# voyage-ai/weaviate

Hardware: AMD Instinct MI355X
Metric: exact kNN QPS (k=10) at 1/2/4/8 GPUs; % of HBM-BW or MFMA roofline (higher is better)
Workload: dtype f32 (exact result; int8 MFMA block-key filter); 1 GPU; 10M x 768 fp32 cosine, k=10, exact flat search (BASELINE configs[2]); corpus_rows=10000000, dims=768, k=10, query_batch=8192, parallelism=corpus sharded over 1 GPU(s), contiguous id ranges, replayed_queries=240

## Files before the change

### weaviate_amd/csrc/q8_kernels.hip

```cpp
#pragma once
#include "batch_row.h"

namespace wv {
namespace {

typedef int i32x4_t __attribute__((ext_vector_type(4)));
typedef int i32x16_t __attribute__((ext_vector_type(16)));
constexpr int Q8_NONE = (int)0x80000000;


template <int OFF>
__device__ __forceinline__ i32x4_t lds_ld16_o(unsigned base) {
    i32x4_t v;
    asm volatile("ds_read_b128 %0, %1 offset:%2" : "=v"(v) : "v"(base), "i"(OFF));
    return v;
}

__global__ void k_allow_bits(const uint64_t* __restrict__ ids, int64_t n, uint64_t id_base, int64_t hiwater,
                             const uint32_t* __restrict__ present, uint32_t* __restrict__ bits,
                             uint32_t* __restrict__ cnt) {
    const int64_t i = (int64_t)blockIdx.x * blockDim.x + threadIdx.x;
    if (i >= n) return;
    const uint64_t id = ids[i];
    if (id < id_base || id - id_base >= (uint64_t)hiwater) return;
// ... 205 lines not shown
        sh += __shfl_xor(sh, o);
        sr += __shfl_xor(sr, o);
    }
    if (lane == 0) {
        const float4 q16 = qinfo16[q];
        qscale[q] = sq;
        qinfo8[q] = make_float4(q16.x, sh, sr, (bad || q16.w != 0.f || !(sh < 1e30f)) ? 1.f : 0.f);
    }
}

}
struct Q8Args {
    const unsigned char* X8;
    const float* sb;
    const float* xnorm2;
    const uint32_t* valid;
    const unsigned char* Q8;
    const float* qscale;
    float* key;
    int64_t ldk;
    int64_t nslots;
    int slots_per_span;
    int nspans;
    int nqg;
    int bq_bits;
    int64_t nq_live = 1ll << 62;
    int prio = 0;
    const uint32_t* qmask = nullptr;
    int64_t qmask_ld = 0;
    int64_t qmask_n = 1;
};
namespace {

template <int NC, int RB, bool ISL2, bool STAG = false, bool BQ = false, int PF = 1, int DBG = 0, bool LIVE = false,
          bool MASK = false>
__global__ __launch_bounds__(512, 2) void k_q8_blockkey(Q8Args a) {
    constexpr int NPB = 2 * NC;
    constexpr int SLOT = RB * NPB * 1024;
    constexpr int P = RB * NPB / 8;
    static_assert((RB * NPB) % 8 == 0, "pieces per slot must split over 8 waves");
    static_assert(RB == 1 || RB == 2, "RB must be 1 or 2");
    constexpr int64_t TILE_B = (int64_t)NPB * 8192;
    constexpr int NT = RB * NC;
    constexpr int P0 = P + 2 + (ISL2 ? 1 : 0) + (MASK ? 1 : 0);
    static_assert(P0 < NC, "the deferred key store must follow the slot's DMA pieces");
    static_assert(PF >= 1 && PF + 1 < NC, "prefetch distance");
    static_assert(!STAG || RB == 2, "the stagger defers a slot's second block");
    static_assert(!BQ || (!ISL2 && !STAG), "BQ: integer maxima, in-order schedule");
    static_assert(!LIVE || (RB == 2 && !STAG && !BQ && DBG == 0), "LIVE: the paired in-order schedule");
    static_assert(!MASK || (RB == 2 && !STAG && !BQ && !ISL2 && DBG == 0), "MASK: paired dot / cosine keys");
    constexpr int X0 = 1;
    constexpr int XE = 2 + (ISL2 ? 2 * RB : 0) + (MASK ? 2 : 0);
    constexpr int NBUF = 3;
    extern __shared__ __attribute__((aligned(16))) unsigned char qsm[];

    const int tid = threadIdx.x;
    const int lane = tid & 63;
    const int wave = __builtin_amdgcn_readfirstlane(tid >> 6);
    const int total = a.nqg * a.nspans;
    const int b = blockIdx.x;
    const int logical = (total % 8 == 0) ? (b % 8) * (total / 8) + (b / 8) : b;
    const int span = logical / a.nqg, grp = logical % a.nqg;
    const bool act = !LIVE || (int64_t)grp * 256 + wave * 32 < a.nq_live;

    i32x4_t Qf[2 * NC];
    const int64_t q0 = (int64_t)grp * 256 + wave * 32;
    if (act) {
        const int j = lane & 15, kq = lane >> 4;
        const unsigned char* qp =
            a.Q8 + (int64_t)grp * TILE_B + (kq >> 1) * 8192 + (wave * 32 + j) * 32 + 16 * (kq & 1);
#pragma unroll
        for (int c = 0; c < NC; c++)
#pragma unroll
            for (int n = 0; n < 2; n++)
                Qf[2 * c + n] = *reinterpret_cast<const i32x4_t*>(qp + (2 * c) * 8192 + n * 16 * 32);
    }
    const float sqA = BQ ? 1.f : a.qscale[q0 + (lane & 15)];
    const float sqB = BQ ? 1.f : a.qscale[q0 + 16 + (lane & 15)];
    constexpr bool PAIR = RB == 2 && !STAG;
    const float sqO = (BQ || !PAIR) ? 1.f : a.qscale[q0 + (lane & 15) + 16 * (lane >> 5)];
    __builtin_amdgcn_s_waitcnt(0x0F70);

    const int64_t s0 = (int64_t)span * a.slots_per_span;
// ... 201 lines not shown
        } else if constexpr (ISL2) {
            float p0, p1;
            reduce(ac, vw_, sb_, xa_, xb_, p0, p1);
            rr[0] = __float_as_uint(p0);
            rr[1] = __float_as_uint(p1);
        } else if (vw == 0xFFFFFFFFu) {
#pragma unroll
            for (int n = 0; n < 2; n++)
                rr[n] = (uint32_t)max(max(max(ac[0][n][0], ac[0][n][1]), max(ac[0][n][2], ac[0][n][3])),
                                      max(max(ac[1][n][0], ac[1][n][1]), max(ac[1][n][2], ac[1][n][3])));
        } else {
#pragma unroll
            for (int n = 0; n < 2; n++) {
                int mi = Q8_NONE;
#pragma unroll
                for (int mm = 0; mm < 2; mm++)
#pragma unroll
                    for (int r = 0; r < 4; r++) mi = max(mi, ((vl >> (16 * mm + r)) & 1u) ? ac[mm][n][r] : Q8_NONE);
                rr[n] = (uint32_t)mi;
            }
        }
        r0 = rr[0];
        r1 = rr[1];
    };
    constexpr uint32_t PNONE = ISL2 ? 0x7f800000u : (uint32_t)Q8_NONE;
    uint32_t pA0 = PNONE, pA1 = PNONE, pB0 = PNONE, pB1 = PNONE;
    float psA = 0.f, psB = 0.f;
    i32x4_t acc[RB][2][2];
    const bool late = STAG && wave >= 4;
    uint32_t dvw = 0;
    float dsb = 0.f;
    f32x4_t dxa = {0.f, 0.f, 0.f, 0.f}, dxb = {0.f, 0.f, 0.f, 0.f};
    if (a.prio && wave >= 4) __builtin_amdgcn_s_setprio(1);
    auto slot_loop = [&](auto actc) {
    constexpr bool ACT = decltype(actc)::value;
    int cur = 0;
    for (int t = 0; t < nsteps; t++) {
        const int nxt = cur == NBUF - 1 ? 0 : cur + 1;
        const int gslot = cur == 0 ? NBUF - 1 : cur - 1;
        const unsigned sbase = ring + (unsigned)(cur * SLOT) + l16;
        const int dma = __builtin_amdgcn_readfirstlane(t + 2 < nsteps ? 1 : 0);
        const unsigned sm = (unsigned)(t & 3);
        uint2 vwv;
        float2 sbv;
        uint2 mw0 = uint2{0u, 0u}, mw1 = uint2{0u, 0u};
        f32x4_t xa[RB], xb[RB];
        if constexpr (!ISL2) {
#pragma unroll
            for (int r = 0; r < RB; r++) xa[r] = xb[r] = f32x4_t{0.f, 0.f, 0.f, 0.f};
        }
        static_for<0, NT>([&](auto ttc) {
            constexpr int tt = decltype(ttc)::value;
            constexpr int rb = tt / NC, c = tt % NC;
            if constexpr (tt == X0 && ACT) {
                asm volatile("ds_read_b64 %0, %1" : "=v"(vwv) : "v"(vring + sm * 16u));
                asm volatile("ds_read_b64 %0, %1" : "=v"(sbv) : "v"(sring + sm * 16u));
                if constexpr (MASK) {
                    const unsigned mb = mring + sm * 256u + (unsigned)((lane & 15) * 8);
                    asm volatile("ds_read_b64 %0, %1" : "=v"(mw0) : "v"(mb));
                    asm volatile("ds_read_b64 %0, %1 offset:128" : "=v"(mw1) : "v"(mb));
                }
                if constexpr (ISL2) {
                    const unsigned xbase = xnring + sm * (unsigned)(RB * 128) + (unsigned)(16 * ((lane >> 4) & 3));
                    xa[0] = lds_ld4f_o<0>(xbase);
                    xb[0] = lds_ld4f_o<64>(xbase);
                    if constexpr (RB == 2) {
// ... 67 lines not shown
            dsb = sbv.y;
            dxa = xa[RB - 1];
            dxb = xb[RB - 1];
        } else if constexpr (PAIR && !(DBG & 4)) {
            if constexpr (ACT) {
                reduce_raw(acc[1], vwv.y, sbv.y, xa[1], xb[1], pB0, pB1, mw1);
                psA = sbv.x;
                psB = sbv.y;
            }
        } else if constexpr (!(DBG & 4)) {
            reduce(acc[RB - 1], RB == 2 ? vwv.y : vwv.x, RB == 2 ? sbv.y : sbv.x, xa[RB - 1], xb[RB - 1], mp0, mp1);
        } else {
#pragma unroll
            for (int r = 0; r < RB; r++)
                dbg_sink ^= acc[r][0][0][0] ^ acc[r][0][1][0] ^ acc[r][1][0][0] ^ acc[r][1][1][0];
        }
        gbp = (s0 + t) * RB + (PAIR ? 0 : RB - 1);
        if (t + 1 < nsteps) {
            if constexpr (DBG != 0) {
                qs_wait_vm_c<0>();
            } else if (t >= 2 && t + 2 < nsteps) {
                qs_wait_vm_c<2 * SPS + P0>();
            } else {
                const int y = (t >= 1 ? stores_in(t - 1) : 0) + stores_in(t) + (t + 2 < nsteps ? P0 : 0);
                qs_wait_vm(y);
            }
            __builtin_amdgcn_s_barrier();
            __builtin_amdgcn_sched_barrier(0);
            if constexpr (ACT) head_reads(ring + (unsigned)(nxt * SLOT) + l16);
        }
        cur = nxt;
    }
    };
    if constexpr (LIVE) {
        if (act) slot_loop(std::true_type{});
        else slot_loop(std::false_type{});
    } else {
        slot_loop(std::true_type{});
    }
    if (nsteps > 0 && !(DBG & 4)) {
        if constexpr (PAIR) {
            finish2(pA0, pA1, pB0, pB1, psA, psB, gbp);
        } else {
            if (late) reduce(acc[RB - 1], dvw, dsb, dxa, dxb, mp0, mp1);
            finish(mp0, mp1, gbp);
        }
    }
    if constexpr ((DBG & 12) != 0) {
        if (a.ldk == -1234567) krow[0] = (float)dbg_sink;
    }
}

template <int NC, int RB, bool ISL2>
__global__ __launch_bounds__(512, 2) void k_q8_blockkey32(Q8Args a) {
    constexpr int SLOT = RB * NC * 1024;
    constexpr int P = RB * NC / 8;
    static_assert((RB * NC) % 8 == 0, "pieces per slot must split over 8 waves");
    constexpr int64_t TILE_B = (int64_t)NC * 8192;
    constexpr int NBUF = 3;
    extern __shared__ __attribute__((aligned(16))) unsigned char qsm[];

    const int tid = threadIdx.x;
    const int lane = tid & 63;
    const int wave = __builtin_amdgcn_readfirstlane(tid >> 6);
    const int li = lane & 31, lh = lane >> 5;
    const int total = a.nqg * a.nspans;
    const int b = blockIdx.x;
    const int logical = (total % 8 == 0) ? (b % 8) * (total / 8) + (b / 8) : b;
    const int span = logical / a.nqg, grp = logical % a.nqg;

    i32x4_t Qf[NC];
    {
        const unsigned char* qp = a.Q8 + (int64_t)grp * TILE_B + (wave * 32 + li) * 32 + 16 * lh;
#pragma unroll
// ... 450 lines not shown
```

### weaviate_amd/csrc/qs_runtime.hip

```cpp
#include "rt_index.h"

int qs_R(int k) { return k + 1 <= 64 ? 2 : k + 1 <= 192 ? 4 : k + 1 <= 448 ? 8 : k + 1 <= 960 ? 16 : 0; }
int qs_R_flat(int k) {
    const int r = qs_R(k);
    return r ? r : k + 1 <= 1984 ? 32 : k + 1 <= 4032 ? 64 : 0;
}

int invert_lists(wv_index* idx, hipStream_t s, const uint32_t* cand, const int32_t* ncand, const int32_t* flags,
                 int64_t cn, int L, int64_t nb) {
    HIPCHK(idx->bmCnt.ensure((size_t)nb * sizeof(uint32_t)));
    HIPCHK(idx->bmOff.ensure((size_t)(nb + 1) * sizeof(uint32_t)));
    HIPCHK(idx->bmPairs.ensure((size_t)cn * L * sizeof(uint32_t)));
    if (idx->bmCnt_zp != idx->bmCnt.p || idx->bmCnt_zb != idx->bmCnt.bytes)
        HIPCHK(hipMemsetAsync(idx->bmCnt.p, 0, idx->bmCnt.bytes, s));
    idx->bmCnt_zp = nullptr;
    const unsigned gw = (unsigned)((cn + 3) / 4);
    k_inv_count<<<gw, 256, 0, s>>>(cand, ncand, flags, (int)cn, L, idx->bmCnt.as<uint32_t>());
    const unsigned nparts = (unsigned)((nb + INV_CHUNK - 1) / INV_CHUNK);
    HIPCHK(idx->bmPart.ensure((size_t)nparts * sizeof(uint32_t)));
    k_inv_part<<<nparts, 1024, 0, s>>>(idx->bmCnt.as<uint32_t>(), nb, idx->bmPart.as<uint32_t>());
    k_inv_scan<<<nparts, 1024, 0, s>>>(idx->bmCnt.as<uint32_t>(), nb, idx->bmPart.as<uint32_t>(),
                                       idx->bmOff.as<uint32_t>());
    k_inv_scatter<<<gw, 256, 0, s>>>(cand, ncand, flags, (int)cn, L, idx->bmOff.as<uint32_t>(),
                                     idx->bmCnt.as<uint32_t>(), idx->bmPairs.as<uint32_t>());
    HIPCHK(hipGetLastError());
    idx->bmCnt_zp = idx->bmCnt.p;
    idx->bmCnt_zb = idx->bmCnt.bytes;
    return WV_OK;
}

int launch_q8_keys(wv_index* idx, hipStream_t s, Q8Args a, int dpb8, bool l2) {
    const int NC8 = dpb8 / 64;
    const int RB = dpb8 <= 768 ? 2 : 1;
    int64_t nspans = 256 / std::gcd(256, a.nqg);
    while ((int64_t)a.nqg * nspans < 256) nspans *= 2;
    if (idx->spans_opt > 0) nspans = idx->spans_opt;
    const int64_t max_sps = ((1ll << 32) - 2 * 256ll * dpb8) / ((int64_t)RB * 32 * dpb8);
    nspans = std::max<int64_t>(nspans, (a.nslots + max_sps - 1) / max_sps);
    if (idx->spans_opt <= 0) {
        const int64_t unit = 256 / std::gcd(256, a.nqg);
        nspans = (nspans + unit - 1) / unit * unit;
    }
    nspans = std::max<int64_t>(1, std::min<int64_t>(nspans, a.nslots));
    const int64_t sps = (a.nslots + nspans - 1) / nspans;
    a.slots_per_span = (int)sps;
    a.nspans = (int)((a.nslots + sps - 1) / sps);
    const size_t lds = (size_t)3 * RB * 2 * NC8 * 1024 + 1024 + (l2 ? (size_t)8 * 4 * RB * 128 : 0);
    dim3 grid((unsigned)((int64_t)a.nqg * a.nspans));
#define WV_Q8K(NCV, RBV, L2V)                                                                                  \
    do {                                                                                                       \
        HIPCHK(hipFuncSetAttribute((const void*)k_q8_blockkey<NCV, RBV, L2V, false, false, 1>,                 \
                                   hipFuncAttributeMaxDynamicSharedMemorySize, (int)lds));                     \
        k_q8_blockkey<NCV, RBV, L2V, false, false, 1><<<grid, 512, lds, s>>>(a);                                \
    } while (0)
#define WV_Q8KN(L2V)                                   \
    switch (NC8) {                                     \
    case 8: WV_Q8K(8, 2, L2V); break;                  \
    case 10: WV_Q8K(10, 2, L2V); break;                \
    case 12: WV_Q8K(12, 2, L2V); break;                \
    case 16: WV_Q8K(16, 1, L2V); break;                \
    case 20: WV_Q8K(20, 1, L2V); break;                \
    case 24: WV_Q8K(24, 1, L2V); break;                \
    default: return set_err(WV_ERR_UNSUPPORTED, "int8 keys: plane width %d", dpb8); \
    }
    if (l2) { WV_Q8KN(true); } else { WV_Q8KN(false); }
#undef WV_Q8KN
#undef WV_Q8K
    HIPCHK(hipGetLastError());
    return WV_OK;
}

bool pqa_keys_route(const wv_index* idx) {
    const bool q8 = idx->q8_planes && (idx->q8_opt || idx->q8_only);
    return idx->pqa_keys && q8 && !idx->q8_only && idx->dpb8 <= 768 && idx->metric != WV_METRIC_L2_SQUARED &&
           !idx->q8_stag && idx->q8_shape != 32 && idx->sel_dbg <= 0;
}

int search_qs(wv_index* idx, hipStream_t s, int64_t nq, int k, int mode, const uint32_t* valid,
                     uint64_t* o_ids, float* o_d, int32_t* o_n, int32_t* o_flags, int phase,
                     float* topA, const float* gA, const float* gE, int W) {
    const int kout = mode == 1 ? k + 1 : k;
    const int NK = idx->dpb / 16;
    const bool q8 = idx->q8_planes && (idx->q8_opt || idx->q8_only);
    const bool q8cp = q8 && idx->q8_only;
    const bool q8wide = q8cp && idx->dpb8 > Q8_MAX_DPB;
    const int NC8 = idx->dpb8 / 64;
    const int RB8 = idx->dpb8 <= 768 ? 2 : 1;
    const int RB = q8 ? RB8 : qs_rb(NK);
    const bool pqa = idx->pqa_valid != nullptr;
    const bool pqk = pqa && pqa_keys_route(idx);
    const bool pqs = pqa && !pqk;
    int R = qs_R_flat(k);
    if (q8) {
        if (idx->q8_R > 0) R = std::max(R, idx->q8_R);
        else R = std::max(R, 8);
    }
    if (pqs) R = std::max(R, idx->pqa_R);
    const int L = 64 * (R - 1);
    const int64_t nslots = std::max<int64_t>(1, (idx->hiwater + 32 * RB - 1) / (32 * RB));
// ... 105 lines not shown
        if (time_it) HIPCHK(hipEventRecord(idx->ev0, s));
#define WV_QS(NKV, L2V)                                                                                        \
    do {                                                                                                       \
        HIPCHK(hipFuncSetAttribute((const void*)k_qs_blockkey<NKV, L2V>, hipFuncAttributeMaxDynamicSharedMemorySize, (int)lds)); \
        k_qs_blockkey<NKV, L2V><<<grid, 512, lds, s>>>(a);                                                     \
    } while (0)
#define WV_QS3(NKV, L2V, D)                                                                                    \
    do {                                                                                                       \
        HIPCHK(hipFuncSetAttribute((const void*)k_qs_blockkey<NKV, L2V, D>, hipFuncAttributeMaxDynamicSharedMemorySize, (int)lds)); \
        k_qs_blockkey<NKV, L2V, D><<<grid, 512, lds, s>>>(a);                                                  \
    } while (0)
#define WV_QSN(L2V)                                    \
    switch (NK) {                                      \
    case 8: WV_QS(8, L2V); break;                      \
    case 16: WV_QS(16, L2V); break;                    \
    case 24: WV_QS(24, L2V); break;                    \
    case 32: WV_QS(32, L2V); break;                    \
    case 40: WV_QS(40, L2V); break;                    \
    default: WV_QS(48, L2V); break;                    \
    }
#define WV_QSW(NKV, L2V, NBV)                                                                                  \
    do {                                                                                                       \
        HIPCHK(hipFuncSetAttribute((const void*)k_qs_blockkey_w4<NKV, L2V, 2, NBV>, hipFuncAttributeMaxDynamicSharedMemorySize, (int)lds)); \
        k_qs_blockkey_w4<NKV, L2V, 2, NBV><<<grid, 256, lds, s>>>(a);                                          \
    } while (0)
#define WV_QSWN(L2V)                                   \
    if (NK == 64) WV_QSW(64, L2V, 4); else WV_QSW(96, L2V, 3);
#define WV_Q8S(NCV, RBV, L2V, STV, PFV)                                                                        \
    do {                                                                                                       \
        HIPCHK(hipFuncSetAttribute((const void*)k_q8_blockkey<NCV, RBV, L2V, STV, false, PFV>, hipFuncAttributeMaxDynamicSharedMemorySize, (int)lds)); \
        k_q8_blockkey<NCV, RBV, L2V, STV, false, PFV><<<grid, 512, lds, s>>>(q8a);                              \
    } while (0)
#define WV_Q8(NCV, RBV, L2V) do { if (idx->q8_pf == 2) WV_Q8S(NCV, RBV, L2V, false, 2); else WV_Q8S(NCV, RBV, L2V, false, 1); } while (0)
#ifdef WV_QS_DBG
#define WV_Q8D(DV)                                                                                             \
    do {                                                                                                       \
        HIPCHK(hipFuncSetAttribute((const void*)k_q8_blockkey<12, 2, false, false, false, 1, DV>, hipFuncAttributeMaxDynamicSharedMemorySize, (int)lds)); \
        k_q8_blockkey<12, 2, false, false, false, 1, DV><<<grid, 512, lds, s>>>(q8a);                           \
    } while (0)
#endif
#define WV_Q8L(NCV, L2V)                                                                                       \
    do {                                                                                                       \
        HIPCHK(hipFuncSetAttribute((const void*)k_q8_blockkey<NCV, 2, L2V, false, false, 1, 0, true>, hipFuncAttributeMaxDynamicSharedMemorySize, (int)lds)); \
        k_q8_blockkey<NCV, 2, L2V, false, false, 1, 0, true><<<grid, 512, lds, s>>>(q8a);                     \
    } while (0)
        const bool q8live = idx->q8_live && cn % QS_QPB != 0;
#define WV_Q8M(NCV, LIVEV)                                                                                     \
    do {                                                                                                       \
        HIPCHK(hipFuncSetAttribute((const void*)k_q8_blockkey<NCV, 2, false, false, false, 1, 0, LIVEV, true>, hipFuncAttributeMaxDynamicSharedMemorySize, (int)lds)); \
        k_q8_blockkey<NCV, 2, false, false, false, 1, 0, LIVEV, true><<<grid, 512, lds, s>>>(q8a);           \
    } while (0)
#define WV_Q8T(NCV, L2V)                                                                                       \
    do {                                                                                                       \
        if constexpr (!L2V) {                                                                                  \
            if (pqk) { if (q8live) WV_Q8M(NCV, true); else WV_Q8M(NCV, false); break; }                       \
        }                                                                                                      \
        if (idx->q8_stag) WV_Q8S(NCV, 2, L2V, true, 1); else if (q8live) WV_Q8L(NCV, L2V); else WV_Q8(NCV, 2, L2V); \
    } while (0)
#define WV_Q8N(L2V)                                    \
    switch (NC8) {                                     \
    case 8: WV_Q8T(8, L2V); break;                     \
    case 10: WV_Q8T(10, L2V); break;                   \
    case 12: WV_Q8T(12, L2V); break;                   \
    case 16: WV_Q8(16, 1, L2V); break;                 \
    case 20: WV_Q8(20, 1, L2V); break;                 \
    default: WV_Q8(24, 1, L2V); break;                 \
    }
        idx->stats.last_route = q8 ? WV_ROUTE_QS_INT8 : w4 ? WV_ROUTE_QS_W4 : WV_ROUTE_QS_BF16;
        if (q8) {
            Q8Args q8a;
            q8a.X8 = idx->X8;
            q8a.sb = idx->sb8;
            q8a.xnorm2 = idx->xnorm2;
            q8a.valid = valid;
            q8a.Q8 = idx->q8Qb.as<unsigned char>();
            q8a.qscale = idx->q8Scale.as<float>();
            q8a.key = a.key;
            q8a.ldk = ldk;
            q8a.nslots = nslots;
            q8a.slots_per_span = a.slots_per_span;
            q8a.nspans = a.nspans;
            q8a.nqg = a.nqg;
            q8a.nq_live = cn;
            q8a.prio = idx->q8_prio;
            if (pqk) {
                q8a.qmask = exv;
                q8a.qmask_ld = idx->pqa_vq;
                q8a.qmask_n = cn;
            }
#ifdef WV_QS_DBG
            if (idx->sel_dbg > 0 && !l2 && NC8 == 12) {
                switch (idx->sel_dbg) {
                case 1: WV_Q8D(1); break;
                case 2: WV_Q8D(2); break;
                case 3: WV_Q8D(3); break;
                case 4: WV_Q8D(4); break;
                case 5: WV_Q8D(5); break;
                case 6: WV_Q8D(6); break;
                case 8: WV_Q8D(8); break;
                case 9: WV_Q8D(9); break;
                default: WV_Q8D(7); break;
                }
            } else
#endif
            const int qg = cn <= 16 ? 1 : 2;
            const bool gemv = idx->q8_gemv && !q8cp && !pqk && cn <= 32 && NC8 <= (qg == 1 ? 24 : 16) && nb < (1ll << 40);
            if (gemv) {
                idx->stats.last_route = WV_ROUTE_Q8_GEMV;
                const unsigned gg = (unsigned)std::max<int64_t>(1, std::min<int64_t>(2048, (nb + 3) / 4));
#define WV_Q8G(NCV, QGV, L2V) k_q8_gemv<NCV, QGV, L2V><<<gg, 256, 0, s>>>(q8a, nb)
#define WV_Q8GQ(NCV, L2V) do { if (qg == 1) WV_Q8G(NCV, 1, L2V); else WV_Q8G(NCV, 2, L2V); } while (0)
#define WV_Q8GN(L2V)                                   \
    switch (NC8) {                                     \
    case 8: WV_Q8GQ(8, L2V); break;                    \
    case 10: WV_Q8GQ(10, L2V); break;                  \
    case 12: WV_Q8GQ(12, L2V); break;                  \
    case 16: WV_Q8GQ(16, L2V); break;                  \
    case 20: WV_Q8G(20, 1, L2V); break;                \
    default: WV_Q8G(24, 1, L2V); break;                \
    }
                if (l2) { WV_Q8GN(true); } else { WV_Q8GN(false); }
#undef WV_Q8GN
#undef WV_Q8GQ
#undef WV_Q8G
            } else if (idx->q8_shape == 32) {
#define WV_Q832(NCV, RBV, L2V)                                                                                \
    do {                                                                                                      \
        HIPCHK(hipFuncSetAttribute((const void*)k_q8_blockkey32<NCV, RBV, L2V>, hipFuncAttributeMaxDynamicSharedMemorySize, (int)lds)); \
        k_q8_blockkey32<NCV, RBV, L2V><<<grid, 512, lds, s>>>(q8a);                                            \
    } while (0)
#define WV_Q832N(L2V)                                  \
    switch (NC8) {                                     \
    case 8: WV_Q832(16, 2, L2V); break;                \
    case 10: WV_Q832(20, 2, L2V); break;               \
    case 12: WV_Q832(24, 2, L2V); break;               \
    case 16: WV_Q832(32, 1, L2V); break;               \
    case 20: WV_Q832(40, 1, L2V); break;               \
    default: WV_Q832(48, 1, L2V); break;               \
    }
                if (l2) { WV_Q832N(true); } else { WV_Q832N(false); }
// ... 19 lines not shown
    case 80: WV_Q8CPW(5, L2V); break;                  \
    default: WV_Q8CPW(6, L2V); break;                  \
    }
                if (l2) { WV_Q8CPN(true); } else { WV_Q8CPN(false); }
#undef WV_Q8CPN
#undef WV_Q8CPW
#undef WV_Q8CP
            } else if (l2) { WV_Q8N(true); } else { WV_Q8N(false); }
        } else if (w4) {
            if (l2) { WV_QSWN(true); } else { WV_QSWN(false); }
#ifdef WV_QS_DBG
        } else if (idx->sel_dbg > 0 && !l2 && NK == 48) {
            switch (idx->sel_dbg) {
            case 1: WV_QS3(48, false, 1); break;
            case 2: WV_QS3(48, false, 2); break;
            case 3: WV_QS3(48, false, 3); break;
            case 4: WV_QS3(48, false, 4); break;
            case 5: WV_QS3(48, false, 5); break;
            case 6: WV_QS3(48, false, 6); break;
            default: WV_QS3(48, false, 7); break;
            }
#endif
        } else if (l2) { WV_QSN(true); } else { WV_QSN(false); }
#undef WV_QSN
#undef WV_QS3
#undef WV_QS
#undef WV_QSWN
#undef WV_QSW
#undef WV_Q8N
#undef WV_Q8T
#undef WV_Q8M
#undef WV_Q8L
#undef WV_Q8S
#undef WV_Q8
        HIPCHK(hipGetLastError());
        if (time_it) { HIPCHK(hipEventRecord(idx->ev1, s)); idx->timed = 1; }
        idx->stats.mfma_launches++;
#ifdef WV_QS_DBG
        if (idx->sel_dbg > 0) {
            HIPCHK(hipMemsetAsync(o_n + c0, 0, (size_t)cn * sizeof(int32_t), s));
            continue;
        }
#endif
        }
        int32_t* flags = phase ? idx->qsFlags.as<int32_t>() : o_flags ? o_flags + c0 : idx->qsFlags.as<int32_t>();
        int32_t* olist = idx->qsList.as<int32_t>() + qc;
        const bool ctr_reset = phase == 0;
        int sel_rc = WV_OK;
        auto sel = [&](int RV, const int32_t* list, const uint32_t* cnt, float* tA) {
            const unsigned gw = (unsigned)((cn + 3) / 4);
            uint32_t* lc = (ctr_reset && !list) ? idx->qscount : nullptr;
            const int RT = qs_R_flat(k);
            if (!list && !pqs && cn <= idx->sel_split_max && RT <= RV && RT <= 8) {
                const int P = (int)std::max<int64_t>(1, std::min<int64_t>(256, (nb + 2047) / 2048));
                const int LV = 64 * (RV - 1);
                const size_t pb = (size_t)cn * P * (k + 1) * sizeof(float);
                if (idx->qsScratch.ensure(pb + (size_t)cn * sizeof(float)) != hipSuccess) {
                    sel_rc = set_err(WV_ERR_HIP, "split selection: %zu bytes of scratch", pb + (size_t)cn * sizeof(float));
                    return;
                }
                float* part = idx->qsScratch.as<float>();
                float* Tq = part + (size_t)cn * P * (k + 1);
                dim3 gp((unsigned)P, (unsigned)cn);
#define WV_SPLIT(RTV)                                                                                             \
    do {                                                                                                          \
        k_sel_part<RTV><<<gp, 64, 0, s>>>(a.key, ldk, nb, k, P, part);                                            \
// ... 372 lines not shown
```

### weaviate_amd/csrc/rt_index.h

```cpp
#pragma once
#include <cerrno>
#include <cpuid.h>
#include <stdarg.h>

#include <algorithm>
#include <cmath>
#include <cstdio>
#include <cstring>
#include <mutex>
#include <atomic>
#include <numeric>
#include <string>
#include <unordered_map>
#include <vector>

#include "../../include/wv_knn.h"
#include "kernels.hip"
#include "bq_kernels.hip"
#include "pq_kernels.hip"
#include "kernels_bf3.hip"
#include "rq_kernels.hip"
#include "gemv_kernels.hip"
#include "qs_kernels.hip"
#include "q8_kernels.hip"
// ... 68 lines not shown
    float* xnorm2 = nullptr;
    uint32_t* present = nullptr;
    uint32_t* d_maxn2 = nullptr;
    uint64_t* codes = nullptr;
    int words = 0;
    unsigned char* bq8 = nullptr;
    int dpb8b = 0;
    int bq8_opt = 1;
    int64_t bq_last_nq = 0, bq_last_nblk = 0, bq_last_blk = 256;
    int scan_window = 1;
    int64_t gather_max = 1 << 20;
    wv_index* sub = nullptr;
    DBuf subSlots;
    DBuf allowIds, allowCnt;
    int64_t bq_nq = 0;
    int bq_R = 0;
    int64_t qt_nq = 0, qt_ld = 0;
    int qt_k = 0, qt_R = 0, qt_trim = 0, qt_rescore = 0, qt_comp = 0, qt_form = 0;
    int pq_m = 0, pq_ks = 0, pq_ds = 0, pq_training_limit = 0, pq_rescore = 1, pq_trained = 0;
    float* pq_centers = nullptr;
    uint32_t* pq_codes = nullptr;
    int use_qs = 0, qs_planes = 0, dpb = 0;
    int exact_filter = 1;
    uint16_t* Xb = nullptr;
    int q8_planes = 0, dpb8 = 0;
    int q8_only = 0;
    int64_t sel_split_max = 512;
    int sel_filter = 1;
    int q8_opt = 1;
    int q8_R = 0;
    int q8_shape = 16;
    int q8_stag = 0;
    int q8_pf = 1;
    int q8_gemv = 1;
    int q8_live = 1;
    int q8_prio = 0;
    int rp_few = 16;
    int bq_fast = 0;
    int q8_filter = 1;
    unsigned char* X8 = nullptr;
    float* sb8 = nullptr;
    uint32_t* qmax8 = nullptr;
    DBuf q8Qb, q8Scale, q8Info, q8Blk;
    uint32_t* qsmax = nullptr;
    uint32_t* qscount = nullptr;
    int has_nonfinite = 0;
    uint64_t replayed_host = 0;
    int timed = 0;
    int timed_total = 0;
    int64_t rq_dbg_nq = 0, rq_dbg_nb = 0;
    int64_t qs_last_nq = 0, qs_last_nb = 0, qs_last_ldk = 0;
    int64_t qs_keys_nq = 0;
    hipEvent_t evt0 = nullptr, evt1 = nullptr;
    float last_eps_scale = 0.f, last_eps_base = 0.f;
    int64_t last_nq = 0;
    int last_KP = 0;
    int rq_bits = 0, rq_D = 0, rq_ready = 0;
    uint16_t* rq_src = nullptr;
    float* rq_sign = nullptr;
    float* rq_round = nullptr;
    void* rq_codes = nullptr;
    unsigned char* rq1_pm = nullptr;
    float4* rq_meta = nullptr;
    int sq_ready = 0, sq_Dq = 0;
    float sq_a = 0.f, sq_b = 0.f, sq_a2 = 0.f, sq_ab = 0.f, sq_ib2 = 0.f;
    uint4* sq_codes = nullptr;
// ... 156 lines not shown
```

### weaviate_amd/csrc/runtime.hip

```cpp
#include "rt_index.h"
#include <cpuid.h>
#include <functional>
#include <map>

static thread_local std::string g_err;

int set_err(int code, const char* fmt, ...) {
    char buf[1024];
    va_list ap;
    va_start(ap, fmt);
    vsnprintf(buf, sizeof(buf), fmt, ap);
    va_end(ap);
    g_err = buf;
    return code;
}


extern "C" const char* wv_last_error(void) { return g_err.c_str(); }

static bool host_has_amxbf16_avx512() {
    unsigned a, b, c, d;
    if (!__get_cpuid_count(7, 0, &a, &b, &c, &d)) return false;
    bool avx512f = (b >> 16) & 1u;
    bool amxbf16 = (d >> 22) & 1u;
// ... 649 lines not shown
    else if (k == "pq8") idx->pq8_opt = value ? 1 : 0;
    else if (k == "q8_gemv") idx->q8_gemv = value ? 1 : 0;
    else if (k == "q8_live") idx->q8_live = value ? 1 : 0;
    else if (k == "q8_prio") idx->q8_prio = value ? 1 : 0;
    else if (k == "sel_split_max") idx->sel_split_max = value;
    else if (k == "rq_mfma") idx->rq_mfma = value ? 1 : 0;
    else if (k == "q8_bm_min") idx->q8_bm_min = value;
    else if (k == "rq_serial") idx->rq_serial = (int)value;
    else if (k == "exact_cap") idx->exact_cap = value ? 1 : 0;
    else if (k == "exact_filter") idx->exact_filter = value ? 1 : 0;
    else if (k == "ef") idx->hnsw_ef = (int)value;
    else if (k == "ef_min") idx->ef_min = (int)value;
    else if (k == "ef_max") idx->ef_max = (int)value;
    else if (k == "ef_factor") idx->ef_factor = (int)value;
    else if (k == "hnsw_rescore") idx->hnsw_rescore = value ? 1 : 0;
    else if (k == "rescore_limit") idx->rescore_limit = (int)value;
    else if (k == "pq_adc") {
        if (value != 1 && value != 2) return set_err(WV_ERR_INVALID, "pq_adc must be 1 or 2");
        idx->pq_adc = (int)value;
    }
    else if (k == "rp_pool") {
        if (value < 1 || value > (1ll << 26)) return set_err(WV_ERR_INVALID, "rp_pool out of range");
        idx->rp_pool = value;
        idx->rpBlk.release(); idx->rpLb.release(); idx->rpQ.release(); idx->rpE.release(); idx->rpVm.release();
    }
    else if (k == "cache") {
        if (value != 0 && value != 1) return set_err(WV_ERR_INVALID, "cache must be 0 or 1");
        idx->cache_opt = (int)value;
    }
    else if (k == "sel_dbg") idx->sel_dbg = (int)value;
    else if (k == "q8") idx->q8_opt = value ? 1 : 0;
    else if (k == "q8_filter") idx->q8_filter = value ? 1 : 0;
    else if (k == "q8_stag") idx->q8_stag = value ? 1 : 0;
    else if (k == "q8_pf") {
        if (value != 1 && value != 2) return set_err(WV_ERR_INVALID, "q8_pf must be 1 or 2");
        idx->q8_pf = (int)value;
    }
    else if (k == "q8_shape") {
        if (value != 16 && value != 32) return set_err(WV_ERR_INVALID, "q8_shape must be 16 or 32");
        idx->q8_shape = (int)value;
    }
    else if (k == "bq8") idx->bq8_opt = value ? 1 : 0;
    else if (k == "pqa") idx->pqa = value ? 1 : 0;
    else if (k == "sel_lower") idx->sel_lower = value ? 1 : 0;
    else if (k == "pqa_alone") idx->pqa_alone = value ? 1 : 0;
    else if (k == "pqa_keys") idx->pqa_keys = value ? 1 : 0;
    else if (k == "bq_fast") idx->bq_fast = value ? 1 : 0;
    else if (k == "rp_few") idx->rp_few = value;
    else if (k == "batch_rows") idx->batch_rows = value ? 1 : 0;
    else if (k == "pqa_split_max") idx->pqa_split_max = std::max<int64_t>(value, 0);
    else if (k == "pqa_budget_mb") idx->pqa_budget_mb = std::max<int64_t>(value, 1);
    else if (k == "scan_window") idx->scan_window = value ? 1 : 0;
    else if (k == "gather_max") {
        if (value < 0 || value > (1ll << 28)) return set_err(WV_ERR_INVALID, "gather_max out of range");
        idx->gather_max = value;
    }
    else if (k == "q8_R") {
        if (value != 0 && value != 2 && value != 4 && value != 8) return set_err(WV_ERR_INVALID, "q8_R must be 0, 2, 4 or 8");
        idx->q8_R = (int)value;
    }
    else if (k == "qgroup") idx->qgroup_opt = (int)value;
    else if (k == "sel_opt") idx->sel_opt = (int)value;
    else return set_err(WV_ERR_INVALID, "unknown option %s", key);
    return WV_OK;
}

// ... 449 lines not shown
        if (idx->codes) idx->codes += lo;
        if (idx->bq8) idx->bq8 += lo * idx->dpb8b;
        idx->id_base += (uint64_t)lo;
    }
    ~ScanWindow() {
        idx->X = X; idx->xnorm2 = xnorm2; idx->present = present; idx->Xb = Xb; idx->X8 = X8; idx->sb8 = sb8;
        idx->codes = codes; idx->bq8 = bq8; idx->hiwater = hiwater; idx->id_base = id_base;
    }
};

static bool window_ok(const wv_index* idx) {
    return idx->compression == WV_COMPRESSION_NONE || idx->compression == WV_COMPRESSION_BQ;
}

static int subindex_build(wv_index* idx, hipStream_t s, const std::vector<uint32_t>& slots) {
    const int64_t n = (int64_t)slots.size();
    if (!idx->sub) {
        wv_config c{};
        c.metric = idx->metric;
        c.dims = idx->dims;
        c.compression = WV_COMPRESSION_NONE;
        c.rescore_limit = -1;
        c.device = idx->device;
        c.variant = idx->variant;
        c.id_base = 0;
        c.root_path = idx->root_path.c_str();
        int rc = wv_index_create(&c, &idx->sub);
        if (rc) return rc;
    }
    wv_index* sb = idx->sub;
    sb->use_qs = idx->use_qs;
    set_dims(sb, idx->dims);
    sb->kernel_opt = idx->kernel_opt; sb->q8_opt = idx->q8_opt; sb->q8_R = idx->q8_R; sb->q8_filter = idx->q8_filter;
    sb->q8_stag = idx->q8_stag; sb->q8_shape = idx->q8_shape; sb->q8_pf = idx->q8_pf; sb->exact_filter = idx->exact_filter; sb->exact_bm = idx->exact_bm; sb->q8_bm = idx->q8_bm; sb->q8_gemv = idx->q8_gemv; sb->q8_live = idx->q8_live; sb->q8_prio = idx->q8_prio; sb->sel_split_max = idx->sel_split_max; sb->q8_bm_min = idx->q8_bm_min;
    sb->exact_cap = idx->exact_cap; sb->replay_par = idx->replay_par; sb->rp_few = idx->rp_few; sb->margin = idx->margin;
    sb->gemv_max = idx->gemv_max; sb->gemv_wg = idx->gemv_wg; sb->exact_multi = idx->exact_multi;
    sb->force_replay = idx->force_replay; sb->qs_force_flag = idx->qs_force_flag; sb->timing = idx->timing;
    sb->hiwater = 0;
    sb->npresent = 0;
    int rc = ensure_capacity(sb, round_up(std::max<int64_t>(n, 1), 256));
    if (rc) return rc;
    HIPCHK(idx->subSlots.ensure((size_t)n * sizeof(uint32_t)));
    HIPCHK(hipMemcpyAsync(idx->subSlots.p, slots.data(), (size_t)n * sizeof(uint32_t), hipMemcpyHostToDevice, s));
    const int64_t n_pad = round_up(n, 256);
    {
        const int64_t per = idx->dpad / 4 + (sb->qs_planes ? idx->dpb / 8 : 0) + 1;
        const int64_t nt = n_pad * per;
        k_gather_rows<<<(unsigned)((nt + 255) / 256), 256, 0, s>>>(idx->X, idx->xnorm2, idx->dpad,
                                                                    sb->qs_planes ? idx->Xb : nullptr, idx->dpb,
                                                                    idx->subSlots.as<uint32_t>(), n, n_pad, sb->X,
                                                                    sb->xnorm2, sb->Xb);
        HIPCHK(hipGetLastError());
    }
    std::vector<uint32_t> bits((size_t)(sb->cap / 32), 0);
    for (int64_t i = 0; i < n; i++) bits[(size_t)(i >> 5)] |= 1u << (i & 31);
    HIPCHK(hipMemcpyAsync(sb->present, bits.data(), bits.size() * sizeof(uint32_t), hipMemcpyHostToDevice, s));
    HIPCHK(hipMemcpyAsync(sb->d_maxn2, idx->d_maxn2, sizeof(uint32_t), hipMemcpyDeviceToDevice, s));
    HIPCHK(hipMemcpyAsync(sb->qsmax, idx->qsmax, 4 * sizeof(uint32_t), hipMemcpyDeviceToDevice, s));
    if (sb->q8_planes) {
        HIPCHK(hipMemsetAsync(sb->qmax8, 0, 4 * sizeof(uint32_t), s));
        k_block_q8<<<(unsigned)(n_pad / 32), 256, 0, s>>>(sb->X, sb->dpad, sb->dims, sb->dpb8, nullptr, 0, sb->X8, sb->sb8,
                                                          sb->qmax8);
        HIPCHK(hipGetLastError());
    }
    HIPCHK(hipStreamSynchronize(s));
    sb->hiwater = n;
    sb->npresent = n;
// ... 698 lines not shown
```

Baseline: 157,500 queries/s.

## Add seam schedule overlapping slot epilogue and next-slot reads in int8 block-key kernel

Adds a SEAM variant of the paired int8 MFMA block-key kernel. It moves the slot barrier and the DMA issue into the middle of the slot's MFMA sequence, prefetches the next slot's first LDS fragments before the boundary, and defers the second block's reduction and the key store into the next slot's early MFMAs. The aim is to hide the barrier, the reduce and the key-write bubble at each slot boundary behind matrix work. It is on by default through the new q8_sched flag. In exchange it adds register pressure from the carried state and makes the wait-count ordering more intricate.

```diff
diff --git a/weaviate_amd/csrc/q8_kernels.hip b/weaviate_amd/csrc/q8_kernels.hip
--- a/weaviate_amd/csrc/q8_kernels.hip
+++ b/weaviate_amd/csrc/q8_kernels.hip
@@ -261,8 +261,20 @@
 };
 namespace {
 
+constexpr int Q8_SEAM_RD = 1, Q8_SEAM_KS = 2;
+constexpr int q8_seam_xb(int nc) { return nc; }
+constexpr bool q8_seam_fits(int nc, bool l2) {
+    const int xb = q8_seam_xb(nc);
+    const int p0 = nc / 2 + 2 + (l2 ? 1 : 0);
+    return xb >= 1 && xb + p0 < 2 * nc && Q8_SEAM_RD < Q8_SEAM_KS && Q8_SEAM_KS <= xb && Q8_SEAM_RD < nc &&
+           Q8_SEAM_KS < nc + 1;
+}
+static_assert(q8_seam_fits(8, false) && q8_seam_fits(8, true) && q8_seam_fits(10, false) && q8_seam_fits(10, true) &&
+                  q8_seam_fits(12, false) && q8_seam_fits(12, true),
+              "SEAM chunk placement");
+
 template <int NC, int RB, bool ISL2, bool STAG = false, bool BQ = false, int PF = 1, int DBG = 0, bool LIVE = false,
-          bool MASK = false>
+          bool MASK = false, bool SEAM = false>
 __global__ __launch_bounds__(512, 2) void k_q8_blockkey(Q8Args a) {
     constexpr int NPB = 2 * NC;
     constexpr int SLOT = RB * NPB * 1024;
@@ -278,6 +290,9 @@
     static_assert(!BQ || (!ISL2 && !STAG), "BQ: integer maxima, in-order schedule");
     static_assert(!LIVE || (RB == 2 && !STAG && !BQ && DBG == 0), "LIVE: the paired in-order schedule");
     static_assert(!MASK || (RB == 2 && !STAG && !BQ && !ISL2 && DBG == 0), "MASK: paired dot / cosine keys");
+    static_assert(!SEAM || (RB == 2 && !STAG && !BQ && !MASK && PF == 1), "SEAM: the paired in-order variants, PF = 1");
+    static_assert(!SEAM || q8_seam_fits(NC, ISL2), "SEAM: group t+2 is issued between the barrier and the slot's end");
+    constexpr int XB = q8_seam_xb(NC), RD = Q8_SEAM_RD, KS = Q8_SEAM_KS;
     constexpr int X0 = 1;
     constexpr int XE = 2 + (ISL2 ? 2 * RB : 0) + (MASK ? 2 : 0);
     constexpr int NBUF = 3;
@@ -545,6 +560,119 @@
     float dsb = 0.f;
     f32x4_t dxa = {0.f, 0.f, 0.f, 0.f}, dxb = {0.f, 0.f, 0.f, 0.f};
     if (a.prio && wave >= 4) __builtin_amdgcn_s_setprio(1);
+    uint32_t cvw = 0;
+    f32x4_t cxa = {0.f, 0.f, 0.f, 0.f}, cxb = {0.f, 0.f, 0.f, 0.f};
+    auto seam_loop = [&](auto actc) {
+    constexpr bool ACT = decltype(actc)::value;
+    static_assert(NT % NB2 == 0, "the fragment sets continue across the slot boundary");
+    int cur = 0;
+    for (int t = 0; t < nsteps; t++) {
+        const int nxt = cur == NBUF - 1 ? 0 : cur + 1;
+        const int gslot = cur == 0 ? NBUF - 1 : cur - 1;
+        const unsigned sbase = ring + (unsigned)(cur * SLOT) + l16;
+        const unsigned snext = ring + (unsigned)(nxt * SLOT) + l16;
+        const int more = __builtin_amdgcn_readfirstlane(t + 1 < nsteps ? 1 : 0);
+        const int dma = __builtin_amdgcn_readfirstlane(t + 2 < nsteps ? 1 : 0);
+        const unsigned sm = (unsigned)(t & 3);
+        uint2 vwv = uint2{0u, 0u};
+        float2 sbv = float2{0.f, 0.f};
+        f32x4_t xa[RB], xb[RB];
+#pragma unroll
+        for (int r = 0; r < RB; r++) xa[r] = xb[r] = f32x4_t{0.f, 0.f, 0.f, 0.f};
+        static_for<0, NT>([&](auto ttc) {
+            constexpr int tt = decltype(ttc)::value;
+            constexpr int rb = tt / NC, c = tt % NC;
+            if constexpr (tt == X0 && ACT) {
+                asm volatile("ds_read_b64 %0, %1" : "=v"(vwv) : "v"(vring + sm * 16u));
+                asm volatile("ds_read_b64 %0, %1" : "=v"(sbv) : "v"(sring + sm * 16u));
+                if constexpr (ISL2) {
+                    const unsigned xbase = xnring + sm * (unsigned)(RB * 128) + (unsigned)(16 * ((lane >> 4) & 3));
+                    xa[0] = lds_ld4f_o<0>(xbase);
+                    xb[0] = lds_ld4f_o<64>(xbase);
+                    xa[1] = lds_ld4f_o<128>(xbase);
+                    xb[1] = lds_ld4f_o<192>(xbase);
+                }
+            }
+            if constexpr (tt + 1 < NT) {
+                if constexpr (ACT) {
+                    constexpr int o1 = ((tt + 1) / NC * NPB + 2 * ((tt + 1) % NC)) * 1024;
+                    B2[(tt + 1) % NB2][0] = lds_ld16_o<o1>(sbase);
+                    B2[(tt + 1) % NB2][1] = lds_ld16_o<o1 + 512>(sbase);
+                }
+                qs_wait_lgkm<2 + (tt == X0 ? XE : 0)>();
+            } else {
+                if (more) {
+                    if constexpr (ACT) {
+                        B2[0][0] = lds_ld16_o<0>(snext);
+                        B2[0][1] = lds_ld16_o<512>(snext);
+                    }
+                    qs_wait_lgkm<2>();
+                } else {
+                    qs_wait_lgkm<0>();
+                }
+            }
+            asm volatile("" : "+v"(B2[tt % NB2][0]), "+v"(B2[tt % NB2][1]));
+            if constexpr (tt == X0 + 1 && ACT) {
+                if constexpr (ISL2) asm volatile("" : "+v"(vwv), "+v"(sbv), "+v"(xa[0]), "+v"(xb[0]), "+v"(xa[1]), "+v"(xb[1]));
+                else asm volatile("" : "+v"(vwv), "+v"(sbv));
+            }
+            __builtin_amdgcn_sched_barrier(0);
+            if constexpr (ACT)
+#pragma unroll
+            for (int m = 0; m < 2; m++)
+#pragma unroll
+                for (int n = 0; n < 2; n++) {
+                    if constexpr (DBG & 2) { acc[rb][m][n] = B2[tt % NB2][m]; continue; }
+                    if constexpr (c == 0)
+                        acc[rb][m][n] = __builtin_amdgcn_mfma_i32_16x16x64_i8(B2[tt % NB2][m], Qf[2 * c + n],
+                                                                              i32x4_t{0, 0, 0, 0}, 0, 0, 0);
+                    else
+                        acc[rb][m][n] = __builtin_amdgcn_mfma_i32_16x16x64_i8(B2[tt % NB2][m], Qf[2 * c + n],
+                                                                              acc[rb][m][n], 0, 0, 0);
+                }
+            if constexpr (tt == RD && !(DBG & 4) && ACT) {
+                if (t > 0) reduce_raw(acc[1], cvw, psB, cxa, cxb, pB0, pB1);
+            }
+            if constexpr (tt == KS && !(DBG & 4)) {
+                if (t > 0) finish2(pA0, pA1, pB0, pB1, psA, psB, gbp);
+            }
+            if constexpr (tt == XB) {
+                __builtin_amdgcn_sched_barrier(0);
+                if (more) {
+                    if constexpr (DBG != 0) {
+                        qs_wait_vm_c<0>();
+                    } else if (t > 0) {
+                        qs_wait_vm_c<1>();
+                    } else {
+                        qs_wait_vm_c<0>();
+                    }
+                    __builtin_amdgcn_s_barrier();
+                }
+                __builtin_amdgcn_sched_barrier(0);
+            }
+            if constexpr (tt > XB && tt <= XB + P0) {
+                if (dma) issue_piece(tt - XB - 1, t + 2, gslot);
+            }
+            if constexpr (tt == NC + 1 && !(DBG & 4) && ACT) reduce_raw(acc[0], vwv.x, sbv.x, xa[0], xb[0], pA0, pA1);
+        });
+        if constexpr (ACT) {
+            psA = sbv.x;
+            psB = sbv.y;
+            cvw = vwv.y;
+            if constexpr (ISL2) {
+                cxa = xa[1];
+                cxb = xb[1];
+            }
+            if constexpr ((DBG & 4) != 0) {
+#pragma unroll
+                for (int r = 0; r < RB; r++)
+                    dbg_sink ^= acc[r][0][0][0] ^ acc[r][0][1][0] ^ acc[r][1][0][0] ^ acc[r][1][1][0];
+            }
+        }
+        gbp = (s0 + t) * RB;
+        cur = nxt;
+    }
+    };
     auto slot_loop = [&](auto actc) {
     constexpr bool ACT = decltype(actc)::value;
     int cur = 0;
@@ -678,14 +806,22 @@
         cur = nxt;
     }
     };
-    if constexpr (LIVE) {
+    if constexpr (SEAM && LIVE) {
+        if (act) seam_loop(std::true_type{});
+        else seam_loop(std::false_type{});
+    } else if constexpr (SEAM) {
+        seam_loop(std::true_type{});
+    } else if constexpr (LIVE) {
         if (act) slot_loop(std::true_type{});
         else slot_loop(std::false_type{});
     } else {
         slot_loop(std::true_type{});
     }
     if (nsteps > 0 && !(DBG & 4)) {
-        if constexpr (PAIR) {
+        if constexpr (SEAM) {
+            if (act) reduce_raw(acc[1], cvw, psB, cxa, cxb, pB0, pB1);
+            finish2(pA0, pA1, pB0, pB1, psA, psB, gbp);
+        } else if constexpr (PAIR) {
             finish2(pA0, pA1, pB0, pB1, psA, psB, gbp);
         } else {
             if (late) reduce(acc[RB - 1], dvw, dsb, dxa, dxb, mp0, mp1);
diff --git a/weaviate_amd/csrc/qs_runtime.hip b/weaviate_amd/csrc/qs_runtime.hip
--- a/weaviate_amd/csrc/qs_runtime.hip
+++ b/weaviate_amd/csrc/qs_runtime.hip
@@ -47,17 +47,25 @@
     a.nspans = (int)((a.nslots + sps - 1) / sps);
     const size_t lds = (size_t)3 * RB * 2 * NC8 * 1024 + 1024 + (l2 ? (size_t)8 * 4 * RB * 128 : 0);
     dim3 grid((unsigned)((int64_t)a.nqg * a.nspans));
+    const bool seam = idx->q8_sched && !idx->q8_stag && idx->q8_pf == 1;
 #define WV_Q8K(NCV, RBV, L2V)                                                                                  \
     do {                                                                                                       \
         HIPCHK(hipFuncSetAttribute((const void*)k_q8_blockkey<NCV, RBV, L2V, false, false, 1>,                 \
                                    hipFuncAttributeMaxDynamicSharedMemorySize, (int)lds));                     \
         k_q8_blockkey<NCV, RBV, L2V, false, false, 1><<<grid, 512, lds, s>>>(a);                                \
     } while (0)
+#define WV_Q8KP(NCV, L2V)                                                                                      \
+    do {                                                                                                       \
+        if (!seam) { WV_Q8K(NCV, 2, L2V); break; }                                                             \
+        HIPCHK(hipFuncSetAttribute((const void*)k_q8_blockkey<NCV, 2, L2V, false, false, 1, 0, false, false, true>, \
+                                   hipFuncAttributeMaxDynamicSharedMemorySize, (int)lds));                     \
+        k_q8_blockkey<NCV, 2, L2V, false, false, 1, 0, false, false, true><<<grid, 512, lds, s>>>(a);          \
+    } while (0)
 #define WV_Q8KN(L2V)                                   \
     switch (NC8) {                                     \
-    case 8: WV_Q8K(8, 2, L2V); break;                  \
-    case 10: WV_Q8K(10, 2, L2V); break;                \
-    case 12: WV_Q8K(12, 2, L2V); break;                \
+    case 8: WV_Q8KP(8, L2V); break;                    \
+    case 10: WV_Q8KP(10, L2V); break;                  \
+    case 12: WV_Q8KP(12, L2V); break;                  \
     case 16: WV_Q8K(16, 1, L2V); break;                \
     case 20: WV_Q8K(20, 1, L2V); break;                \
     case 24: WV_Q8K(24, 1, L2V); break;                \
@@ -65,6 +73,7 @@
     }
     if (l2) { WV_Q8KN(true); } else { WV_Q8KN(false); }
 #undef WV_Q8KN
+#undef WV_Q8KP
 #undef WV_Q8K
     HIPCHK(hipGetLastError());
     return WV_OK;
@@ -236,9 +245,20 @@
         k_q8_blockkey<NCV, RBV, L2V, STV, false, PFV><<<grid, 512, lds, s>>>(q8a);                              \
     } while (0)
 #define WV_Q8(NCV, RBV, L2V) do { if (idx->q8_pf == 2) WV_Q8S(NCV, RBV, L2V, false, 2); else WV_Q8S(NCV, RBV, L2V, false, 1); } while (0)
+#define WV_Q8E(NCV, L2V, LIVEV)                                                                                \
+    do {                                                                                                       \
+        HIPCHK(hipFuncSetAttribute((const void*)k_q8_blockkey<NCV, 2, L2V, false, false, 1, 0, LIVEV, false, true>, hipFuncAttributeMaxDynamicSharedMemorySize, (int)lds)); \
+        k_q8_blockkey<NCV, 2, L2V, false, false, 1, 0, LIVEV, false, true><<<grid, 512, lds, s>>>(q8a);        \
+    } while (0)
+        const bool q8seam = idx->q8_sched && !idx->q8_stag && idx->q8_pf == 1;
 #ifdef WV_QS_DBG
 #define WV_Q8D(DV)                                                                                             \
     do {                                                                                                       \
+        if (q8seam) {                                                                                          \
+            HIPCHK(hipFuncSetAttribute((const void*)k_q8_blockkey<12, 2, false, false, false, 1, DV, false, false, true>, hipFuncAttributeMaxDynamicSharedMemorySize, (int)lds)); \
+            k_q8_blockkey<12, 2, false, false, false, 1, DV, false, false, true><<<grid, 512, lds, s>>>(q8a);  \
+            break;                                                                                             \
+        }                                                                                                      \
         HIPCHK(hipFuncSetAttribute((const void*)k_q8_blockkey<12, 2, false, false, false, 1, DV>, hipFuncAttributeMaxDynamicSharedMemorySize, (int)lds)); \
         k_q8_blockkey<12, 2, false, false, false, 1, DV><<<grid, 512, lds, s>>>(q8a);                           \
     } while (0)
@@ -259,7 +279,10 @@
         if constexpr (!L2V) {                                                                                  \
             if (pqk) { if (q8live) WV_Q8M(NCV, true); else WV_Q8M(NCV, false); break; }                       \
         }                                                                                                      \
-        if (idx->q8_stag) WV_Q8S(NCV, 2, L2V, true, 1); else if (q8live) WV_Q8L(NCV, L2V); else WV_Q8(NCV, 2, L2V); \
+        if (idx->q8_stag) WV_Q8S(NCV, 2, L2V, true, 1);                                                        \
+        else if (q8seam) { if (q8live) WV_Q8E(NCV, L2V, true); else WV_Q8E(NCV, L2V, false); }                 \
+        else if (q8live) WV_Q8L(NCV, L2V);                                                                     \
+        else WV_Q8(NCV, 2, L2V);                                                                               \
     } while (0)
 #define WV_Q8N(L2V)                                    \
     switch (NC8) {                                     \
@@ -293,7 +316,8 @@
                 q8a.qmask_n = cn;
             }
 #ifdef WV_QS_DBG
-            if (idx->sel_dbg > 0 && !l2 && NC8 == 12) {
+            const bool q8dbg = idx->sel_dbg > 0 && !l2 && NC8 == 12;
+            if (q8dbg) {
                 switch (idx->sel_dbg) {
                 case 1: WV_Q8D(1); break;
                 case 2: WV_Q8D(2); break;
@@ -305,11 +329,14 @@
                 case 9: WV_Q8D(9); break;
                 default: WV_Q8D(7); break;
                 }
-            } else
+            }
+#else
+            const bool q8dbg = false;
 #endif
             const int qg = cn <= 16 ? 1 : 2;
             const bool gemv = idx->q8_gemv && !q8cp && !pqk && cn <= 32 && NC8 <= (qg == 1 ? 24 : 16) && nb < (1ll << 40);
-            if (gemv) {
+            if (q8dbg) {
+            } else if (gemv) {
                 idx->stats.last_route = WV_ROUTE_Q8_GEMV;
                 const unsigned gg = (unsigned)std::max<int64_t>(1, std::min<int64_t>(2048, (nb + 3) / 4));
 #define WV_Q8G(NCV, QGV, L2V) k_q8_gemv<NCV, QGV, L2V><<<gg, 256, 0, s>>>(q8a, nb)
@@ -395,6 +422,7 @@
 #undef WV_Q8M
 #undef WV_Q8L
 #undef WV_Q8S
+#undef WV_Q8E
 #undef WV_Q8
         HIPCHK(hipGetLastError());
         if (time_it) { HIPCHK(hipEventRecord(idx->ev1, s)); idx->timed = 1; }
diff --git a/weaviate_amd/csrc/rt_index.h b/weaviate_amd/csrc/rt_index.h
--- a/weaviate_amd/csrc/rt_index.h
+++ b/weaviate_amd/csrc/rt_index.h
@@ -124,6 +124,7 @@
     int q8_shape = 16;
     int q8_stag = 0;
     int q8_pf = 1;
+    int q8_sched = 1;
     int q8_gemv = 1;
     int q8_live = 1;
     int q8_prio = 0;
diff --git a/weaviate_amd/csrc/runtime.hip b/weaviate_amd/csrc/runtime.hip
--- a/weaviate_amd/csrc/runtime.hip
+++ b/weaviate_amd/csrc/runtime.hip
@@ -705,6 +705,7 @@
     else if (k == "q8") idx->q8_opt = value ? 1 : 0;
     else if (k == "q8_filter") idx->q8_filter = value ? 1 : 0;
     else if (k == "q8_stag") idx->q8_stag = value ? 1 : 0;
+    else if (k == "q8_sched") idx->q8_sched = value ? 1 : 0;
     else if (k == "q8_pf") {
         if (value != 1 && value != 2) return set_err(WV_ERR_INVALID, "q8_pf must be 1 or 2");
         idx->q8_pf = (int)value;
@@ -1220,7 +1221,7 @@
     sb->use_qs = idx->use_qs;
     set_dims(sb, idx->dims);
     sb->kernel_opt = idx->kernel_opt; sb->q8_opt = idx->q8_opt; sb->q8_R = idx->q8_R; sb->q8_filter = idx->q8_filter;
-    sb->q8_stag = idx->q8_stag; sb->q8_shape = idx->q8_shape; sb->q8_pf = idx->q8_pf; sb->exact_filter = idx->exact_filter; sb->exact_bm = idx->exact_bm; sb->q8_bm = idx->q8_bm; sb->q8_gemv = idx->q8_gemv; sb->q8_live = idx->q8_live; sb->q8_prio = idx->q8_prio; sb->sel_split_max = idx->sel_split_max; sb->q8_bm_min = idx->q8_bm_min;
+    sb->q8_stag = idx->q8_stag; sb->q8_shape = idx->q8_shape; sb->q8_pf = idx->q8_pf; sb->q8_sched = idx->q8_sched; sb->exact_filter = idx->exact_filter; sb->exact_bm = idx->exact_bm; sb->q8_bm = idx->q8_bm; sb->q8_gemv = idx->q8_gemv; sb->q8_live = idx->q8_live; sb->q8_prio = idx->q8_prio; sb->sel_split_max = idx->sel_split_max; sb->q8_bm_min = idx->q8_bm_min;
     sb->exact_cap = idx->exact_cap; sb->replay_par = idx->replay_par; sb->rp_few = idx->rp_few; sb->margin = idx->margin;
     sb->gemv_max = idx->gemv_max; sb->gemv_wg = idx->gemv_wg; sb->exact_multi = idx->exact_multi;
     sb->force_replay = idx->force_replay; sb->qs_force_flag = idx->qs_force_flag; sb->timing = idx->timing;
```

Measured after the change: 160,000 queries/s (median of 6 runs). 1.02x the previous value.
